# lgalke/aae-recommender

Hardware: AMD Instinct MI355X
Metric: train docs/sec at |items|=100k h=200 (higher is better)
Workload: dtype f32; 1 GPU; C3 PubMed-scale synthetic Bags: |items|=100000, hidden=200, code=50, fp32, batch=100 docs/GPU/step, full partial_fit (ae+disc+gen, 4 Adam) inside the AdversarialAutoEncoder.fit epoch loop (permutation batches of a corpus resident in HBM); n_items=100000, n_hidden=200, n_code=50, batch_per_gpu=100, global_batch=100, cond_inc=0, rng=device, parallelism=dp1

## Files before the change

### aae-recommender_amd/csrc/aae_abi.hip

```cpp
#include <hip/hip_runtime.h>
#include <hip/hip_ext.h>
#include <math.h>
#include <stdio.h>
#include <stdlib.h>
#include <string.h>

#include <algorithm>
#include <string>
#include <vector>

#include "../../include/aaerec_hip.h"
#include "gemm_f32.h"
#include "kernels.h"
#include "dec_fused.h"
#include "dec_fused_bf16.h"
#include "dec_crit_x3.h"
#include "rank_x3.h"
#include "chain.h"
#include "chain4.h"
#include "chain16x3.h"
#include "cond_embed.h"
#include "w1_update.h"

using namespace aae;
// ... 116 lines not shown
            m->bucket_wide_ok = hipFuncSetAttribute(reinterpret_cast<const void*>(tile_bucket_wide_kernel), hipFuncAttributeMaxDynamicSharedMemorySize, maxlds - 16384) == hipSuccess;
            {
                hipFuncAttributes fa;
                static bool told = false;
                if (m->bucket_wide_ok && !told && hipFuncGetAttributes(&fa, reinterpret_cast<const void*>(tile_bucket_wide_kernel)) == hipSuccess && fa.numRegs < 121) {
                    told = true;
                    fprintf(stderr, "aaerec: tile_bucket_wide_kernel allocates %d vector registers, not the 128 it claims to keep its CU to itself (buckets.h)\n", fa.numRegs);
                }
                (void)hipGetLastError();
            }
            if (e1 != hipSuccess || e2 != hipSuccess || e3 != hipSuccess || e4 != hipSuccess) m->fused_ok = false;
            if (m->bf16 &&
                (hipFuncSetAttribute(reinterpret_cast<const void*>(dec_fused_bf16_kernel<4>), hipFuncAttributeMaxDynamicSharedMemorySize, maxlds) != hipSuccess ||
                 hipFuncSetAttribute(reinterpret_cast<const void*>(dec_fused_bf16_kernel<7>), hipFuncAttributeMaxDynamicSharedMemorySize, maxlds) != hipSuccess ||
                 hipFuncSetAttribute(reinterpret_cast<const void*>(dec_fused_bf16_kernel<13>), hipFuncAttributeMaxDynamicSharedMemorySize, maxlds) != hipSuccess))
                m->fused_ok = false;
        }
    }
    m->late_enabled = !m->opt.no_late_join;
    m->early_enabled = true;
    m->early_any = m->opt.early_any;
    m->rank_ok = m->fused_ok && m->use_chain4 && !m->vae && !m->opt.no_rank_fused && rank_set_attributes();
    m->w1_big_lds = hipFuncSetAttribute(reinterpret_cast<const void*>(w1_item_update_kernel), hipFuncAttributeMaxDynamicSharedMemorySize,
                                        (int)(sizeof(int) * w1_items_lds_words(16384))) == hipSuccess;
    (void)hipGetLastError();
    m->grad_scale = 1.f;
    m->rng_row0 = 0; m->rng_global = 0;
    m->Gt = m->G.p;
    m->split_ok = false; m->opt_pending = false; m->side = nullptr; m->ev_crit = m->ev_opt = nullptr;
    m->split_wgs = std::max(1, (m->n_cu * 5) / 8);
    m->pf_armed = m->pf_built = m->pf_pending = false; m->pf_step = -1; m->hstep = 0; m->flushed_hstep = -1; m->ev_head = m->ev_pf = nullptr;
    bool side_ok = false;
    if (cfg->grad_mode == AAE_GRAD_FUSED) {
        int lo = 0, hi = 0;
        const unsigned evflags = hipEventDisableTiming | hipEventDisableSystemFence;
        side_ok = hipDeviceGetStreamPriorityRange(&lo, &hi) == hipSuccess &&
                  hipStreamCreateWithPriority(&m->side, hipStreamNonBlocking, lo) == hipSuccess &&
                  hipEventCreateWithFlags(&m->ev_crit, evflags) == hipSuccess &&
                  hipEventCreateWithFlags(&m->ev_opt, evflags) == hipSuccess &&
                  hipEventCreateWithFlags(&m->ev_head, evflags) == hipSuccess &&
                  hipEventCreateWithFlags(&m->ev_pf, evflags) == hipSuccess &&
                  hipEventCreateWithFlags(&m->ev_bk, evflags) == hipSuccess &&
                  hipEventCreateWithFlags(&m->ev_end, evflags) == hipSuccess;
        if (!side_ok) {
            if (m->side) (void)hipStreamDestroy(m->side);
            m->side = nullptr;
        }
        (void)hipGetLastError();
    }
    if (side_ok && m->fused_ok && m->bf16 && m->split_wgs > 0 &&
        (size_t)((m->N + kBU - 1) / kBU) * kBU * bf_stride(4) <= (size_t)m->R * m->ldn) {
        m->split_ok = hipFuncSetAttribute(reinterpret_cast<const void*>(dec_fused_bf16_kernel<4, kDecCrit>), hipFuncAttributeMaxDynamicSharedMemorySize, 160 * 1024) == hipSuccess
                && hipFuncSetAttribute(reinterpret_cast<const void*>(dec_fused_bf16_kernel<7, kDecCrit>), hipFuncAttributeMaxDynamicSharedMemorySize, 160 * 1024) == hipSuccess
                && hipFuncSetAttribute(reinterpret_cast<const void*>(dec_fused_bf16_kernel<13, kDecCrit>), hipFuncAttributeMaxDynamicSharedMemorySize, 160 * 1024) == hipSuccess
                && hipFuncSetAttribute(reinterpret_cast<const void*>(dec_fused_bf16_kernel<4, kDecOpt>), hipFuncAttributeMaxDynamicSharedMemorySize, 160 * 1024) == hipSuccess
                && hipFuncSetAttribute(reinterpret_cast<const void*>(dec_fused_bf16_kernel<7, kDecOpt>), hipFuncAttributeMaxDynamicSharedMemorySize, 160 * 1024) == hipSuccess
                && hipFuncSetAttribute(reinterpret_cast<const void*>(dec_fused_bf16_kernel<13, kDecOpt>), hipFuncAttributeMaxDynamicSharedMemorySize, 160 * 1024) == hipSuccess;
        (void)hipGetLastError();
    }
    if (side_ok && m->fused_ok && m->split_wgs > 0 && 
        (size_t)((m->N + kTI - 1) / kTI) * kTI * (size_t)std::min(m->R, 16 * kMB) * sizeof(float) < (size_t)0x7FFFFFF0u) {
        bool ok = true;
        ok = ok && aae_attr2(reinterpret_cast<const void*>(dec_fused_kernel<4, kDecCrit>), reinterpret_cast<const void*>(dec_fused_kernel<4, kDecCrit, true>), hipFuncAttributeMaxDynamicSharedMemorySize, 160 * 1024) == hipSuccess
                && aae_attr2(reinterpret_cast<const void*>(dec_fused_kernel<7, kDecCrit>), reinterpret_cast<const void*>(dec_fused_kernel<7, kDecCrit, true>), hipFuncAttributeMaxDynamicSharedMemorySize, 160 * 1024) == hipSuccess
                && aae_attr2(reinterpret_cast<const void*>(dec_fused_kernel<13, kDecCrit>), reinterpret_cast<const void*>(dec_fused_kernel<13, kDecCrit, true>), hipFuncAttributeMaxDynamicSharedMemorySize, 160 * 1024) == hipSuccess
                && aae_attr2(reinterpret_cast<const void*>(dec_fused_kernel<4, kDecOpt>), reinterpret_cast<const void*>(dec_fused_kernel<4, kDecOpt, true>), hipFuncAttributeMaxDynamicSharedMemorySize, 160 * 1024) == hipSuccess
                && aae_attr2(reinterpret_cast<const void*>(dec_fused_kernel<7, kDecOpt>), reinterpret_cast<const void*>(dec_fused_kernel<7, kDecOpt, true>), hipFuncAttributeMaxDynamicSharedMemorySize, 160 * 1024) == hipSuccess
                && aae_attr2(reinterpret_cast<const void*>(dec_fused_kernel<13, kDecOpt>), reinterpret_cast<const void*>(dec_fused_kernel<13, kDecOpt, true>), hipFuncAttributeMaxDynamicSharedMemorySize, 160 * 1024) == hipSuccess
                && aae_attr2(reinterpret_cast<const void*>(dec_fused_kernel<4, kDecOptAcc>), reinterpret_cast<const void*>(dec_fused_kernel<4, kDecOptAcc, true>), hipFuncAttributeMaxDynamicSharedMemorySize, 160 * 1024) == hipSuccess
                && aae_attr2(reinterpret_cast<const void*>(dec_fused_kernel<7, kDecOptAcc>), reinterpret_cast<const void*>(dec_fused_kernel<7, kDecOptAcc, true>), hipFuncAttributeMaxDynamicSharedMemorySize, 160 * 1024) == hipSuccess
                && aae_attr2(reinterpret_cast<const void*>(dec_fused_kernel<13, kDecOptAcc>), reinterpret_cast<const void*>(dec_fused_kernel<13, kDecOptAcc, true>), hipFuncAttributeMaxDynamicSharedMemorySize, 160 * 1024) == hipSuccess
                && hipFuncSetAttribute(reinterpret_cast<const void*>(dec_opt_blocks_kernel<4>), hipFuncAttributeMaxDynamicSharedMemorySize, 160 * 1024) == hipSuccess
                && hipFuncSetAttribute(reinterpret_cast<const void*>(dec_opt_blocks_kernel<7>), hipFuncAttributeMaxDynamicSharedMemorySize, 160 * 1024) == hipSuccess
                && hipFuncSetAttribute(reinterpret_cast<const void*>(dec_opt_blocks_kernel<13>), hipFuncAttributeMaxDynamicSharedMemorySize, 160 * 1024) == hipSuccess;
        if (!m->bf16) m->split_ok = ok;
        m->x3_ok = ok
                && aae_attr2(reinterpret_cast<const void*>(dec_crit_x3_kernel<4>), reinterpret_cast<const void*>(dec_crit_x3_kernel<4, false, false, true>), hipFuncAttributeMaxDynamicSharedMemorySize, 160 * 1024) == hipSuccess
                && aae_attr2(reinterpret_cast<const void*>(dec_crit_x3_kernel<7>), reinterpret_cast<const void*>(dec_crit_x3_kernel<7, false, false, true>), hipFuncAttributeMaxDynamicSharedMemorySize, 160 * 1024) == hipSuccess
                && aae_attr2(reinterpret_cast<const void*>(dec_crit_x3_kernel<13>), reinterpret_cast<const void*>(dec_crit_x3_kernel<13, false, false, true>), hipFuncAttributeMaxDynamicSharedMemorySize, 160 * 1024) == hipSuccess
                && hipFuncSetAttribute(reinterpret_cast<const void*>(dec_crit_x3_kernel<13, true>), hipFuncAttributeMaxDynamicSharedMemorySize, 160 * 1024) == hipSuccess
                && aae_attr2(reinterpret_cast<const void*>(dec_opt_blocks_x3_kernel<4>), reinterpret_cast<const void*>(dec_opt_blocks_x3_kernel<4, false, true>), hipFuncAttributeMaxDynamicSharedMemorySize, 160 * 1024) == hipSuccess
                && aae_attr2(reinterpret_cast<const void*>(dec_opt_blocks_x3_kernel<7>), reinterpret_cast<const void*>(dec_opt_blocks_x3_kernel<7, false, true>), hipFuncAttributeMaxDynamicSharedMemorySize, 160 * 1024) == hipSuccess
                && aae_attr2(reinterpret_cast<const void*>(dec_opt_blocks_x3_kernel<13>), reinterpret_cast<const void*>(dec_opt_blocks_x3_kernel<13, false, true>), hipFuncAttributeMaxDynamicSharedMemorySize, 160 * 1024) == hipSuccess
                && hipFuncSetAttribute(reinterpret_cast<const void*>(dec_opt_blocks_x3_kernel<13, true>), hipFuncAttributeMaxDynamicSharedMemorySize, 160 * 1024) == hipSuccess;
        (void)hipGetLastError();
        if (m->bf16) {
            m->bf16_x3 = m->x3_ok && ok;
            if (!m->bf16_x3) m->x3_ok = false;
            else m->split_ok = true;
            m->bf16_one = m->bf16_x3
                && aae_attr2(reinterpret_cast<const void*>(dec_crit_x3_kernel<4, false, true>), reinterpret_cast<const void*>(dec_crit_x3_kernel<4, false, true, true>), hipFuncAttributeMaxDynamicSharedMemorySize, 160 * 1024) == hipSuccess
                && aae_attr2(reinterpret_cast<const void*>(dec_crit_x3_kernel<7, false, true>), reinterpret_cast<const void*>(dec_crit_x3_kernel<7, false, true, true>), hipFuncAttributeMaxDynamicSharedMemorySize, 160 * 1024) == hipSuccess
                && aae_attr2(reinterpret_cast<const void*>(dec_crit_x3_kernel<13, false, true>), reinterpret_cast<const void*>(dec_crit_x3_kernel<13, false, true, true>), hipFuncAttributeMaxDynamicSharedMemorySize, 160 * 1024) == hipSuccess
                && aae_attr2(reinterpret_cast<const void*>(dec_opt_x3_kernel<4, true>), reinterpret_cast<const void*>(dec_opt_x3_kernel<4, true, true>), hipFuncAttributeMaxDynamicSharedMemorySize, 160 * 1024) == hipSuccess
                && aae_attr2(reinterpret_cast<const void*>(dec_opt_x3_kernel<7, true>), reinterpret_cast<const void*>(dec_opt_x3_kernel<7, true, true>), hipFuncAttributeMaxDynamicSharedMemorySize, 160 * 1024) == hipSuccess
                && aae_attr2(reinterpret_cast<const void*>(dec_opt_x3_kernel<13, true>), reinterpret_cast<const void*>(dec_opt_x3_kernel<13, true, true>), hipFuncAttributeMaxDynamicSharedMemorySize, 160 * 1024) == hipSuccess
                && aae_attr2(reinterpret_cast<const void*>(dec_opt_x3_kernel<4>), reinterpret_cast<const void*>(dec_opt_x3_kernel<4, false, true>), hipFuncAttributeMaxDynamicSharedMemorySize, 160 * 1024) == hipSuccess
                && aae_attr2(reinterpret_cast<const void*>(dec_opt_x3_kernel<7>), reinterpret_cast<const void*>(dec_opt_x3_kernel<7, false, true>), hipFuncAttributeMaxDynamicSharedMemorySize, 160 * 1024) == hipSuccess
                && aae_attr2(reinterpret_cast<const void*>(dec_opt_x3_kernel<13>), reinterpret_cast<const void*>(dec_opt_x3_kernel<13, false, true>), hipFuncAttributeMaxDynamicSharedMemorySize, 160 * 1024) == hipSuccess;
            (void)hipGetLastError();
        }
        if (m->x3_ok) {
            const int ntiles = (m->N + 31) / 32;
            const double t_tile = (3.3 + 0.0131 * m->h) * (m->bf16_one ? 0.87 : 1.0);
            int w = (int)(ntiles * t_tile / (m->bf16_one ? 165.0 : 82.0) / 8.0 + 0.5) * 8;
            w = std::max(w, std::min(ntiles, m->bf16_one ? 48 : 64));
            const int cap = m->late_enabled ? m->n_cu * 15 / 32 : m->n_cu * 9 / 16;
            m->split_wgs = std::max(1, std::min(w, cap));
        }
    }
    hipStream_t s = S(stream);
    hipError_t e = hipMemsetAsync(arena_dev, 0, need, s);
    if (e != hipSuccess) { delete m; return fail(AAE_EHIP, std::string("hipMemsetAsync: ") + hipGetErrorString(e)); }
    struct { Ten* t; int col; } ones[] = {{&m->eh1, m->h}, {&m->eh2, m->h}, {&m->zc, m->cp}, {&m->dh1, m->h},
                                           {&m->dh2, m->h}, {&m->zin, m->c}, {&m->xh1, m->h}, {&m->xh2, m->h}};
    for (auto& o : ones)
        hipLaunchKernelGGL(fill_col_kernel, dim3(((int)o.t->rows + 255) / 256), dim3(256), 0, s, o.t->p, (int)o.t->ld,
                           (int)o.t->rows, o.col, 1.0f);
    OptScalars hs[4]; memset(hs, 0, sizeof(hs));
    for (int i = 0; i < 4; ++i) {
        hs[i].t = 0; hs[i].is_sgd = cfg->optimizer == AAE_OPT_SGD;
        hs[i].lr = (i == O_ENC || i == O_DEC) ? (double)cfg->gen_lr : (double)cfg->reg_lr;
        hs[i].neg_step_size = 0.f; hs[i].bc2_sqrt = 1.f; hs[i].inv_bc2_sqrt = 1.f;
    }
    e = hipMemcpyAsync(m->sc, hs, sizeof(hs), hipMemcpyHostToDevice, s);
    if (e == hipSuccess) e = hipStreamSynchronize(s);
    if (e != hipSuccess) { delete m; return fail(AAE_EHIP, std::string("init: ") + hipGetErrorString(e)); }
    *out = m;
    return AAE_OK;
}

#ifdef W1_TS
int aae_debug_w1_ts(unsigned long long* out, int n) {
    return (int)hipMemcpyFromSymbol(out, HIP_SYMBOL(aae::w1_ts), sizeof(unsigned long long) * (size_t)n);
}
#endif
int aae_destroy(aae_handle h) {
    if (!h) return AAE_OK;
    if (h->side) {
        (void)hipStreamSynchronize(h->side);
        (void)hipStreamDestroy(h->side);
    }
    if (h->dp_scratch) (void)hipFree(h->dp_scratch);
    if (h->cnt_host) (void)hipHostFree(h->cnt_host);
    if (h->ev_crit) (void)hipEventDestroy(h->ev_crit);
    if (h->ev_opt) (void)hipEventDestroy(h->ev_opt);
    if (h->ev_head) (void)hipEventDestroy(h->ev_head);
    if (h->ev_pf) (void)hipEventDestroy(h->ev_pf);
    if (h->ev_bk) (void)hipEventDestroy(h->ev_bk);
    if (h->ev_end) (void)hipEventDestroy(h->ev_end);
    if (h->prof_ev) {
        for (int k = 0; k < AAE_K_N; ++k)
            for (auto& pr : h->prof_ev[k]) { (void)hipEventDestroy(pr.first); (void)hipEventDestroy(pr.second); }
        delete[] h->prof_ev;
    }
    delete h;
    return AAE_OK;
}


int aae_profile_enable(aae_handle h, int on) {
    if (!h) return fail(AAE_EINVAL, "handle is NULL");
    if (on && !h->prof_ev) h->prof_ev = new std::vector<std::pair<hipEvent_t, hipEvent_t>>[AAE_K_N];
    h->prof_on = on != 0;
    h->prof_mask = on == 1 ? ~0u : ((unsigned)on >> 1);
    return AAE_OK;
}
// ... 138 lines not shown
```

### aae-recommender_amd/csrc/abi_output_layer.h

```cpp
#pragma once

extern "C" {

int aae_ae_decode_backward(aae_handle m, const float* zc_dev, int64_t zc_ld, const aae_rng_inject* inj,
                           float* dzc_out, void* stream) {
    if (!m) return fail(AAE_EINVAL, "handle is NULL");
    if (m->phase != 1) return fail(AAE_ESTATE, "aae_ae_decode_backward without aae_ae_encode");
    remember_inject(m, inj, false);
    hipStream_t s = S(stream);
    const int B = m->rows, N = m->N, h = m->h, cp = m->cp;
    if (zc_dev) TRY(stage_zc(m, zc_dev, zc_ld, B, s));
    const uint8_t* mk2 = m->inj.masks_dev[2];
    const uint8_t* mk3 = m->inj.masks_dev[3];
    if (m->only_output_layer) {  }
    else if (m->use_chain) { if (!m->dec_hidden_done) TRY(chain_dec_hidden(m, true, B, s)); }
    else TRY(decoder_hidden_forward(m, true, mk2, mk3, B, s));
    TRY(join_output_layer(m, s));
    const float gscale = m->grad_scale / ((float)B * (float)N);
    DropSpec d1 = make_drop(m, 0, true, mk2, nullptr, B, h, 2);
    DropSpec d2 = make_drop(m, 1, true, mk3, nullptr, B, h, 3);
    const int nblk = m->have_batch ? row_blocks(m) : 1;
    const int Bb = (B + nblk - 1) / nblk;
    const bool win = x3_big_span(m->N, m->ldh);
    const size_t fused_lds = out_bf16(m) ? dec_fused_bf16_lds_bytes(m->fused_nb ? m->fused_nb : 13) : dec_fused_lds_bytes(Bb, h);
// ... 75 lines not shown
                        break;
                    }
                } else switch (m->fused_nb) {
                    case 4: { if (win) hipExtLaunchKernelGGL((dec_fused_kernel<4, kDecCrit, true>), dim3(grid), dim3(kNT), (uint32_t)fused_lds, s, start, stop, 0, b); else hipExtLaunchKernelGGL((dec_fused_kernel<4, kDecCrit>), dim3(grid), dim3(kNT), (uint32_t)fused_lds, s, start, stop, 0, b); } break;
                    case 7: { if (win) hipExtLaunchKernelGGL((dec_fused_kernel<7, kDecCrit, true>), dim3(grid), dim3(kNT), (uint32_t)fused_lds, s, start, stop, 0, b); else hipExtLaunchKernelGGL((dec_fused_kernel<7, kDecCrit>), dim3(grid), dim3(kNT), (uint32_t)fused_lds, s, start, stop, 0, b); } break;
                    default: { if (win) hipExtLaunchKernelGGL((dec_fused_kernel<13, kDecCrit, true>), dim3(grid), dim3(kNT), (uint32_t)fused_lds, s, start, stop, 0, b); else hipExtLaunchKernelGGL((dec_fused_kernel<13, kDecCrit>), dim3(grid), dim3(kNT), (uint32_t)fused_lds, s, start, stop, 0, b); } break;
                }
                LAUNCHCHK("dec_fused (critical launch)");
                if (r == nblk - 1) HIPCHK(hipStreamWaitEvent(m->side, stop, 0));
            }
            const int g2 = std::min(ntiles, std::min(m->split_wgs, m->n_cu));
            bool late_launched = false;
            constexpr bool no_obk = false, no_opt_x3 = false;
            const bool one_opt = nblk > 1 && !out_bf16(m) && !no_obk && ntiles <= kOBT * m->n_cu &&
                                 dec_opt_blocks_lds_bytes(Bb) <= 160 * 1024;
            constexpr bool no_obk_x3 = false;
            if (nblk > 1 && !out_bf16(m) && m->x3_ok && !no_opt_x3 && !no_obk_x3 && !no_obk && m->dh2f.p) {
                DecFusedArgs b = fa;
                b.nblk = nblk; b.Bb = Bb;
                hipLaunchKernelGGL(dh2_frag_kernel, dim3((B + kXCH - 1) / kXCH, m->fused_nb), dim3(128), 0, m->side, m->dh2.p, m->ldh, B,
                                   reinterpret_cast<u32x4_t*>(m->dh2f.p), b.one_term);
                b.acc = m->dh2f.p;
                const int wg_cap = ntiles >= 4096 ? m->n_cu * 7 / 8 : m->n_cu * 3 / 4;
                const int by_tiles = ntiles < 384 ? std::max(32, std::min(m->n_cu / 2, ntiles / 3))
                                                  : std::max(m->n_cu / 2, std::min(wg_cap, (int)(ntiles / 16.3 / 8.0 + 0.5) * 8));
                const int g3 = std::max(1, std::min(by_tiles, std::min(ntiles, m->n_cu)));
                const int rounds = (ntiles + g3 * kXBT - 1) / (g3 * kXBT);
                b.tpp = g3 * rounds;
                const uint32_t lds3 = (uint32_t)dec_opt_blocks_x3_lds_bytes();
                hipEvent_t start = nullptr, stop = nullptr;
                (void)prof_pair(m, AAE_K_DEC_OPT, &start, &stop);
                if (ts_obk && m->fused_nb == 13) {
                    hipExtLaunchKernelGGL((dec_opt_blocks_x3_kernel<13, true>), dim3(g3), dim3(kNT), lds3, m->side, start, stop, 0, b);
                    HIPCHK(hipStreamSynchronize(m->side));
                    unsigned long long t[128];
                    HIPCHK(hipMemcpy(t, ts_dev, sizeof(t), hipMemcpyDeviceToHost));
                    for (int w = 0; w < 2; ++w) {
                        fprintf(stderr, "[dec_opt_blocks_x3 wave %d, steps 8..15, us: products | split | to the next barrier;  spare wave: - | split | requests | wait for the slot | to the next barrier]", w ? 12 : 0);
                        for (int q = 0; q < 8; ++q) {
                            const unsigned long long* u = t + 64 * w + 4 * q;
                            if (w == 0) fprintf(stderr, "  %.2f %.2f %.2f", (u[1] - u[0]) * 0.01, (u[2] - u[1]) * 0.01, q < 7 ? ((double)u[4] - (double)u[2]) * 0.01 : 0.0);
                            else fprintf(stderr, "  %.2f %.2f %.2f %.2f", (u[1] - u[0]) * 0.01, (u[2] - u[1]) * 0.01, (u[3] - u[2]) * 0.01, q < 7 ? ((double)u[4] - (double)u[3]) * 0.01 : 0.0);
                        }
                        fprintf(stderr, "\n");
                    }
                    for (int k = 0; k < 2; ++k) {
                        const unsigned long long* u = t + (k ? 96 : 32);
                        fprintf(stderr, "[dec_opt_blocks_x3 step %d: every wave's arrival at the step's closing barrier, us after wave 0 finished its products]", k ? 12 : 9);
                        for (int w = 0; w < 16; ++w) fprintf(stderr, " %.2f", ((double)u[w] - (double)u[16]) * 0.01);
                        fprintf(stderr, "\n");
                    }
                } else
                switch (m->fused_nb) {
                    case 4: { if (win) hipExtLaunchKernelGGL((dec_opt_blocks_x3_kernel<4, false, true>), dim3(g3), dim3(kNT), lds3, m->side, start, stop, 0, b); else hipExtLaunchKernelGGL((dec_opt_blocks_x3_kernel<4>), dim3(g3), dim3(kNT), lds3, m->side, start, stop, 0, b); } break;
                    case 7: { if (win) hipExtLaunchKernelGGL((dec_opt_blocks_x3_kernel<7, false, true>), dim3(g3), dim3(kNT), lds3, m->side, start, stop, 0, b); else hipExtLaunchKernelGGL((dec_opt_blocks_x3_kernel<7>), dim3(g3), dim3(kNT), lds3, m->side, start, stop, 0, b); } break;
                    default: { if (win) hipExtLaunchKernelGGL((dec_opt_blocks_x3_kernel<13, false, true>), dim3(g3), dim3(kNT), lds3, m->side, start, stop, 0, b); else hipExtLaunchKernelGGL((dec_opt_blocks_x3_kernel<13>), dim3(g3), dim3(kNT), lds3, m->side, start, stop, 0, b); } break;
                }
                LAUNCHCHK("dec_opt_blocks_x3");
            } else if (one_opt) {
                DecFusedArgs b = fa;
                b.nblk = nblk; b.Bb = Bb;
                const int g3 = std::max(std::min(g2, ntiles), (ntiles + kOBT - 1) / kOBT);
                const uint32_t lds3 = (uint32_t)dec_opt_blocks_lds_bytes(Bb);
                hipEvent_t start = nullptr, stop = nullptr;
                (void)prof_pair(m, AAE_K_DEC_OPT, &start, &stop);
                switch (m->fused_nb) {
                    case 4: hipExtLaunchKernelGGL((dec_opt_blocks_kernel<4>), dim3(g3), dim3(kNT), lds3, m->side, start, stop, 0, b); break;
                    case 7: hipExtLaunchKernelGGL((dec_opt_blocks_kernel<7>), dim3(g3), dim3(kNT), lds3, m->side, start, stop, 0, b); break;
                    default: hipExtLaunchKernelGGL((dec_opt_blocks_kernel<13>), dim3(g3), dim3(kNT), lds3, m->side, start, stop, 0, b); break;
                }
                LAUNCHCHK("dec_opt_blocks");
            } else
            for (int r = 0; r < nblk; ++r) {
                DecFusedArgs b = block_args(r);
                if (nblk > 1) { b.acc = m->Gacc.p; b.gradV3 = r == nblk - 1 ? nullptr : m->Gacc.p; }
                hipEvent_t start = nullptr, stop = nullptr;
                (void)prof_pair(m, AAE_K_DEC_OPT, &start, &stop);
                if (out_bf16(m)) switch (m->fused_nb) {
                    case 4: hipExtLaunchKernelGGL((dec_fused_bf16_kernel<4, kDecOpt>), dim3(g2), dim3(kBT), (uint32_t)fused_lds, m->side, start, stop, 0, b); break;
                    case 7: hipExtLaunchKernelGGL((dec_fused_bf16_kernel<7, kDecOpt>), dim3(g2), dim3(kBT), (uint32_t)fused_lds, m->side, start, stop, 0, b); break;
                    default: hipExtLaunchKernelGGL((dec_fused_bf16_kernel<13, kDecOpt>), dim3(g2), dim3(kBT), (uint32_t)fused_lds, m->side, start, stop, 0, b); break;
                } else if (r == 0 && nblk == 1 && m->x3_ok && !no_opt_x3) {
                    const uint32_t lds_nat = (uint32_t)dec_opt_x3_lds_bytes();
                    const uint32_t lds3 = m->bf16_one ? std::max(lds_nat, 150u * 1024u) : lds_nat;
                    if (late) { b.dh2 = m->dh2s.p; b.sc = m->sc_snap; late_launched = true; }
                    if (m->bf16_one) switch (m->fused_nb) {
                    case 4: { if (win) hipExtLaunchKernelGGL((dec_opt_x3_kernel<4, true, true>), dim3(g2), dim3(kNT), lds3, m->side, start, stop, 0, b); else hipExtLaunchKernelGGL((dec_opt_x3_kernel<4, true>), dim3(g2), dim3(kNT), lds3, m->side, start, stop, 0, b); } break;
                    case 7: { if (win) hipExtLaunchKernelGGL((dec_opt_x3_kernel<7, true, true>), dim3(g2), dim3(kNT), lds3, m->side, start, stop, 0, b); else hipExtLaunchKernelGGL((dec_opt_x3_kernel<7, true>), dim3(g2), dim3(kNT), lds3, m->side, start, stop, 0, b); } break;
                    default: { if (win) hipExtLaunchKernelGGL((dec_opt_x3_kernel<13, true, true>), dim3(g2), dim3(kNT), lds3, m->side, start, stop, 0, b); else hipExtLaunchKernelGGL((dec_opt_x3_kernel<13, true>), dim3(g2), dim3(kNT), lds3, m->side, start, stop, 0, b); } break;
                    } else
                    switch (m->fused_nb) {
                    case 4: { if (win) hipExtLaunchKernelGGL((dec_opt_x3_kernel<4, false, true>), dim3(g2), dim3(kNT), lds3, m->side, start, stop, 0, b); else hipExtLaunchKernelGGL((dec_opt_x3_kernel<4>), dim3(g2), dim3(kNT), lds3, m->side, start, stop, 0, b); } break;
                    case 7: { if (win) hipExtLaunchKernelGGL((dec_opt_x3_kernel<7, false, true>), dim3(g2), dim3(kNT), lds3, m->side, start, stop, 0, b); else hipExtLaunchKernelGGL((dec_opt_x3_kernel<7>), dim3(g2), dim3(kNT), lds3, m->side, start, stop, 0, b); } break;
                    default: { if (win) hipExtLaunchKernelGGL((dec_opt_x3_kernel<13, false, true>), dim3(g2), dim3(kNT), lds3, m->side, start, stop, 0, b); else hipExtLaunchKernelGGL((dec_opt_x3_kernel<13>), dim3(g2), dim3(kNT), lds3, m->side, start, stop, 0, b); } break;
                    }
                } else if (r == 0) switch (m->fused_nb) {
                    case 4: { if (win) hipExtLaunchKernelGGL((dec_fused_kernel<4, kDecOpt, true>), dim3(g2), dim3(kNT), (uint32_t)fused_lds, m->side, start, stop, 0, b); else hipExtLaunchKernelGGL((dec_fused_kernel<4, kDecOpt>), dim3(g2), dim3(kNT), (uint32_t)fused_lds, m->side, start, stop, 0, b); } break;
                    case 7: { if (win) hipExtLaunchKernelGGL((dec_fused_kernel<7, kDecOpt, true>), dim3(g2), dim3(kNT), (uint32_t)fused_lds, m->side, start, stop, 0, b); else hipExtLaunchKernelGGL((dec_fused_kernel<7, kDecOpt>), dim3(g2), dim3(kNT), (uint32_t)fused_lds, m->side, start, stop, 0, b); } break;
                    default: { if (win) hipExtLaunchKernelGGL((dec_fused_kernel<13, kDecOpt, true>), dim3(g2), dim3(kNT), (uint32_t)fused_lds, m->side, start, stop, 0, b); else hipExtLaunchKernelGGL((dec_fused_kernel<13, kDecOpt>), dim3(g2), dim3(kNT), (uint32_t)fused_lds, m->side, start, stop, 0, b); } break;
                } else switch (m->fused_nb) {
                    case 4: { if (win) hipExtLaunchKernelGGL((dec_fused_kernel<4, kDecOptAcc, true>), dim3(g2), dim3(kNT), (uint32_t)fused_lds, m->side, start, stop, 0, b); else hipExtLaunchKernelGGL((dec_fused_kernel<4, kDecOptAcc>), dim3(g2), dim3(kNT), (uint32_t)fused_lds, m->side, start, stop, 0, b); } break;
                    case 7: { if (win) hipExtLaunchKernelGGL((dec_fused_kernel<7, kDecOptAcc, true>), dim3(g2), dim3(kNT), (uint32_t)fused_lds, m->side, start, stop, 0, b); else hipExtLaunchKernelGGL((dec_fused_kernel<7, kDecOptAcc>), dim3(g2), dim3(kNT), (uint32_t)fused_lds, m->side, start, stop, 0, b); } break;
                    default: { if (win) hipExtLaunchKernelGGL((dec_fused_kernel<13, kDecOptAcc, true>), dim3(g2), dim3(kNT), (uint32_t)fused_lds, m->side, start, stop, 0, b); else hipExtLaunchKernelGGL((dec_fused_kernel<13, kDecOptAcc>), dim3(g2), dim3(kNT), (uint32_t)fused_lds, m->side, start, stop, 0, b); } break;
                }
                LAUNCHCHK("dec_fused (optimiser launch)");
            }
            TRY(side_done(m, m->ev_opt));
            m->opt_pending = true;
            m->late_ok = late_launched;
            m->last_out_split = true; m->side_ordered = true;
            if (m->only_output_layer && m->pf_armed && m->mark2 && m->lazy) TRY(launch_prefetch(m, false));
        } else
        {
            m->last_out_split = false; m->side_ordered = false;
            ProfScope ps(m, AAE_K_DEC_FUSED, s);
            const size_t bf_lds = dec_fused_bf16_lds_bytes(m->fused_nb ? m->fused_nb : 13);
            if (m->bf16) switch (m->fused_nb) {
                case 4: hipLaunchKernelGGL(dec_fused_bf16_kernel<4>, dim3(grid), dim3(kBT), bf_lds, s, fa); break;
                case 7: hipLaunchKernelGGL(dec_fused_bf16_kernel<7>, dim3(grid), dim3(kBT), bf_lds, s, fa); break;
                default: hipLaunchKernelGGL(dec_fused_bf16_kernel<13>, dim3(grid), dim3(kBT), bf_lds, s, fa); break;
            } else switch (m->fused_nb) {
                case 4: { if (win) hipLaunchKernelGGL((dec_fused_kernel<4, kDecFused, true>), dim3(grid), dim3(kNT), fused_lds, s, fa); else hipLaunchKernelGGL((dec_fused_kernel<4>), dim3(grid), dim3(kNT), fused_lds, s, fa); } break;
                case 7: { if (win) hipLaunchKernelGGL((dec_fused_kernel<7, kDecFused, true>), dim3(grid), dim3(kNT), fused_lds, s, fa); else hipLaunchKernelGGL((dec_fused_kernel<7>), dim3(grid), dim3(kNT), fused_lds, s, fa); } break;
                default: { if (win) hipLaunchKernelGGL((dec_fused_kernel<13, kDecFused, true>), dim3(grid), dim3(kNT), fused_lds, s, fa); else hipLaunchKernelGGL((dec_fused_kernel<13>), dim3(grid), dim3(kNT), fused_lds, s, fa); } break;
            }
        }
        LAUNCHCHK("dec_fused");
        if (want_ts) {
            unsigned long long t[128];
            HIPCHK(hipStreamSynchronize(s));
            HIPCHK(hipMemcpy(t, ts_dev, sizeof(t), hipMemcpyDeviceToHost));
            if (m->last_out_split && ts_obk) {  }
            else if (m->last_out_split)
                fprintf(stderr, "[dec_crit_x3 tile 5] barrier=%.2f S0=%.2f GEMM1=%.2f BCE=%.2f GEMM3=%.2f | wg 0: prologue=%.2f loop=%.2f (%llu tiles, %.2f each) epilogue=%.2f us\n",
                        (t[14] - t[0]) * 0.01, (t[1] - t[14]) * 0.01, (t[2] - t[1]) * 0.01, (t[3] - t[2]) * 0.01, (t[4] - t[3]) * 0.01,
                        (t[11] - t[10]) * 0.01, (t[7] - t[11]) * 0.01, t[13], (t[7] - t[11]) * 0.01 / (double)(t[13] ? t[13] : 1),
                        (t[12] - t[7]) * 0.01);
            else {
            if (out_bf16(m))
                for (int k = 0; k < 5; ++k) {
                    fprintf(stderr, "[dec_fused_bf16 arrivals at barrier %d, us after the unit's start]", k);
                    for (int w = 0; w < 16; ++w) fprintf(stderr, " %.2f", ((double)t[16 + 16 * k + w] - (double)t[0]) * 0.01);
                    fprintf(stderr, "\n");
                }
            fprintf(stderr, "[dec_fused tile 5] S0=%.2f GEMM1+BCE0=%.2f entries=%.2f GEMM2+GEMM3=%.2f S5=%.2f | tile=%.2f us, %.0f shader clocks -> %.2f GHz\n",
                    (t[1] - t[0]) * 0.01, (t[2] - t[1]) * 0.01, (t[3] - t[2]) * 0.01, (t[4] - t[3]) * 0.01,
                    (t[6] - t[4]) * 0.01, (t[6] - t[0]) * 0.01, (double)(t[9] - t[8]),
                    (double)(t[9] - t[8]) / ((t[6] - t[0]) * 10.0));
            if (out_bf16(m)) fprintf(stderr, "[dec_fused_bf16 S0] barrier A=%.2f work=%.2f barrier B=%.2f us\n", (t[14] - t[0]) * 0.01, (t[15] - t[14]) * 0.01, (t[1] - t[15]) * 0.01);
            fprintf(stderr, "[dec_fused wg 0] prologue=%.2f loop=%.2f (%llu tiles, %.2f each) epilogue=%.2f us\n",
                    (t[11] - t[10]) * 0.01, (t[7] - t[11]) * 0.01, t[13], (t[7] - t[11]) * 0.01 / (double)(t[13] ? t[13] : 1),
                    (t[12] - t[7]) * 0.01);
            }
        }
        float* part = m->slabs.p + (size_t)304 * fa.slab_stride;
        const size_t n4 = (size_t)B * m->ldh / 4;
        if (m->only_output_layer && crit_slabs <= 64) {
            hipLaunchKernelGGL(slab_partial_kernel, dim3((unsigned)((n4 + 255) / 256), 1), dim3(256), 0, s, m->slabs.p, crit_slabs,
                               fa.slab_stride, n4, m->da2.p, (size_t)0, m->bce_partials, n_loss_partials,
                               1.0f / ((float)B * (float)N), m->losses, 0);
            LAUNCHCHK("slabs -> da2");
            m->phase = 2;
            return AAE_OK;
        }
        hipLaunchKernelGGL(slab_partial_kernel, dim3((unsigned)((n4 + 255) / 256), 16), dim3(256), 0, s, m->slabs.p, crit_slabs,
                           fa.slab_stride, n4, part, fa.slab_stride, m->bce_partials, n_loss_partials,
                           1.0f / ((float)B * (float)N), m->losses, 0);
        if (m->only_output_layer) {
            hipLaunchKernelGGL(slab_partial_kernel, dim3((unsigned)((n4 + 255) / 256), 1), dim3(256), 0, s, part, 16,
                               fa.slab_stride, n4, m->da2.p, (size_t)0, (const float*)nullptr, 0, 0.f, m->losses, 0);
            LAUNCHCHK("slab_partial -> da2");
            m->phase = 2;
            return AAE_OK;
        }
        if (m->use_chain) {
            chain_part = part; chain_stride = fa.slab_stride;
        } else {
// ... 112 lines not shown
```

### aae-recommender_amd/csrc/dec_crit_x3.h

```cpp
#pragma once
#include "dec_fused_bf16.h"

namespace aae {

typedef short s16x4_t __attribute__((ext_vector_type(4)));

__device__ __forceinline__ void split3_pair(float a, float b, unsigned& p1, unsigned& p2, unsigned& p3, bool one) {
    x3_split_pair(a, b, p1, p2, p3);
    if (one) { p2 = 0u; p3 = 0u; }
}
__device__ __forceinline__ f32x4 mfma_x3(const bf16x8 (&a)[3], const bf16x8 (&b)[3], f32x4 c) { return x3_mfma(a, b, c); }
template <bool ONE>
__device__ __forceinline__ f32x4 mfma_xt(const bf16x8 (&a)[3], const bf16x8 (&b)[3], f32x4 c) {
    if constexpr (ONE) return __builtin_amdgcn_mfma_f32_16x16x32_bf16(a[0], b[0], c, 0, 0, 0);
    else return x3_mfma(a, b, c);
}

__host__ __device__ constexpr int x3_stride(int kc) { return 16 * kc + 8; }
__device__ __forceinline__ bf16x8 x3_frag(const unsigned* img, int row, int S, int kc, int fk) {
    return __builtin_bit_cast(bf16x8, *reinterpret_cast<const u32x4_t*>(img + row * S + 16 * kc + 4 * fk));
}
constexpr int kXRS = 33;
constexpr int kXT = 32;

// ... 709 lines not shown
        for (int j = 0; j < kXBT; ++j) { acc[j][0] = (f32x4){0.f, 0.f, 0.f, 0.f}; acc[j][1] = (f32x4){0.f, 0.f, 0.f, 0.f}; }
        int q = 0;
        bf16x8 dB[KR][3];
        for (int ch = 0; ch < nch; ++ch) {
            if (mult && (ch == 0 || !(a.dbg_skip & 0x4000))) {
                const u32x4_t* F = reinterpret_cast<const u32x4_t*>(a.acc) + (((size_t)ch * NB + cb) * KR * 3) * 64 + lane;
#pragma unroll
                for (int kc = 0; kc < KR; ++kc)
#pragma unroll
                    for (int t = 0; t < 3; ++t) dB[kc][t] = __builtin_bit_cast(bf16x8, F[(kc * 3 + t) * 64]);
#pragma unroll
                for (int kc = 0; kc < KR; ++kc)
#pragma unroll
                    for (int t = 0; t < 3; ++t) {
                        u32x4_t v = __builtin_bit_cast(u32x4_t, dB[kc][t]);
                        asm volatile("" : "+v"(v));
                        dB[kc][t] = __builtin_bit_cast(bf16x8, v);
                    }
            }
#pragma unroll
            for (int j = 0; j < kXBT; ++j) {
                if (j >= nt) break;
                int oz;
                asm volatile("v_mov_b32 %0, 0" : "=v"(oz));
                const int lz = lane + oz;
                lds_barrier();
                const bool stamp = stamp_wg && (wave == 0 || wave == NM) && q >= 8 && q < 16;
                unsigned long long* tsq = a.ts + (wave ? 64 : 0) + (q - 8) * 4;
                if (stamp) tsq[0] = wall_clock64();
                if (mult && !(a.dbg_skip & 0x1000)) {
                    const int tq = (lz >> 2) & 3, tp = lz & 3, g = lz >> 4;
                    const unsigned* img = gB + (q & 1) * 3 * IMG;
#pragma unroll
                    for (int nb2 = 0; nb2 < 2; ++nb2) {
                        if (nb2 < nb_lo || nb2 >= nb_hi) continue;
                        f32x4 c = acc[j][nb2];
                        const unsigned* base = img + nb2 * (kXCH * 8) + (tq | ((g & 1) << 2) | ((g >> 1) << 4)) * 8 + 2 * tp;
#pragma unroll
                        for (int kc = 0; kc < KR; ++kc) {
                            bf16x8 ga[3];
#pragma unroll
                            for (int t = 0; t < 3; ++t) {
                                const unsigned* pb = base + t * IMG + 32 * kc * 8;
                                const s16x4_t lo = __builtin_amdgcn_ds_read_tr16_b64_v4i16((s16x4_t __attribute__((address_space(3)))*)(pb));
                                const s16x4_t hi = __builtin_amdgcn_ds_read_tr16_b64_v4i16((s16x4_t __attribute__((address_space(3)))*)(pb + 8 * 8));
                                typedef short s16x8_t __attribute__((ext_vector_type(8)));
                                const s16x8_t v = {lo[0], lo[1], lo[2], lo[3], hi[0], hi[1], hi[2], hi[3]};
                                ga[t] = __builtin_bit_cast(bf16x8, v);
                            }
                            c = mfma_x3(ga, dB[kc], c);
                        }
                        acc[j][nb2] = c;
                    }
                }
                if (stamp) tsq[1] = wall_clock64();
                if (splitter && q + 1 < Q) split_write(q + 1, j + 1 < nt ? ch : ch + 1, slot_read(q + 1));
                if (!mult) request(q + kXRing);
                if (stamp) tsq[2] = wall_clock64();
                if (!mult) {
                    asm volatile("s_waitcnt vmcnt(%0)" :: "n"(NS * (kXRing - 2)) : "memory");
                    if (stamp) tsq[3] = wall_clock64();
                }
                if (TS && stamp_wg && (q == 9 || q == 12)) { a.ts[(q == 9 ? 32 : 96) + wave] = wall_clock64(); if (wave == 0) a.ts[(q == 9 ? 48 : 112)] = tsq[1]; }
                ++q;
            }
        }
        asm volatile("s_waitcnt vmcnt(0)" ::: "memory");
        lds_barrier();
        if (mult) {
#pragma unroll
            for (int j = 0; j < kXBT; ++j)
#pragma unroll
                for (int nb2 = 0; nb2 < 2; ++nb2)
                    if (nb2 >= nb_lo && nb2 < nb_hi) {
#pragma unroll
                        for (int rr = 0; rr < 4; ++rr) os[j * (kTI * kSO) + (16 * nb2 + 4 * fk + rr) * kSO + 16 * cb + fr] = acc[j][nb2][rr];
                    }
        }
        lds_barrier();
        optimiser();
    }
}

}
```

Before: 434,100 docs/s.

## Add warp-specialized decoder optimiser kernel with dedicated loader waves prefetching tiles

```diff
diff --git a/aae-recommender_amd/csrc/aae_abi.hip b/aae-recommender_amd/csrc/aae_abi.hip
--- a/aae-recommender_amd/csrc/aae_abi.hip
+++ b/aae-recommender_amd/csrc/aae_abi.hip
@@ -222,7 +222,10 @@
                 && aae_attr2(reinterpret_cast<const void*>(dec_opt_blocks_x3_kernel<4>), reinterpret_cast<const void*>(dec_opt_blocks_x3_kernel<4, false, true>), hipFuncAttributeMaxDynamicSharedMemorySize, 160 * 1024) == hipSuccess
                 && aae_attr2(reinterpret_cast<const void*>(dec_opt_blocks_x3_kernel<7>), reinterpret_cast<const void*>(dec_opt_blocks_x3_kernel<7, false, true>), hipFuncAttributeMaxDynamicSharedMemorySize, 160 * 1024) == hipSuccess
                 && aae_attr2(reinterpret_cast<const void*>(dec_opt_blocks_x3_kernel<13>), reinterpret_cast<const void*>(dec_opt_blocks_x3_kernel<13, false, true>), hipFuncAttributeMaxDynamicSharedMemorySize, 160 * 1024) == hipSuccess
-                && hipFuncSetAttribute(reinterpret_cast<const void*>(dec_opt_blocks_x3_kernel<13, true>), hipFuncAttributeMaxDynamicSharedMemorySize, 160 * 1024) == hipSuccess;
+                && hipFuncSetAttribute(reinterpret_cast<const void*>(dec_opt_blocks_x3_kernel<13, true>), hipFuncAttributeMaxDynamicSharedMemorySize, 160 * 1024) == hipSuccess
+                && aae_attr2(reinterpret_cast<const void*>(dec_opt_ld_x3_kernel<4>), reinterpret_cast<const void*>(dec_opt_ld_x3_kernel<4, true>), hipFuncAttributeMaxDynamicSharedMemorySize, 160 * 1024) == hipSuccess
+                && aae_attr2(reinterpret_cast<const void*>(dec_opt_ld_x3_kernel<7>), reinterpret_cast<const void*>(dec_opt_ld_x3_kernel<7, true>), hipFuncAttributeMaxDynamicSharedMemorySize, 160 * 1024) == hipSuccess
+                && aae_attr2(reinterpret_cast<const void*>(dec_opt_ld_x3_kernel<13>), reinterpret_cast<const void*>(dec_opt_ld_x3_kernel<13, true>), hipFuncAttributeMaxDynamicSharedMemorySize, 160 * 1024) == hipSuccess;
         (void)hipGetLastError();
         if (m->bf16) {
             m->bf16_x3 = m->x3_ok && ok;
diff --git a/aae-recommender_amd/csrc/abi_output_layer.h b/aae-recommender_amd/csrc/abi_output_layer.h
--- a/aae-recommender_amd/csrc/abi_output_layer.h
+++ b/aae-recommender_amd/csrc/abi_output_layer.h
@@ -181,7 +181,7 @@
                     default: hipExtLaunchKernelGGL((dec_fused_bf16_kernel<13, kDecOpt>), dim3(g2), dim3(kBT), (uint32_t)fused_lds, m->side, start, stop, 0, b); break;
                 } else if (r == 0 && nblk == 1 && m->x3_ok && !no_opt_x3) {
                     const uint32_t lds_nat = (uint32_t)dec_opt_x3_lds_bytes();
-                    const uint32_t lds3 = m->bf16_one ? std::max(lds_nat, 150u * 1024u) : lds_nat;
+                    const uint32_t lds3 = m->bf16_one ? std::max(lds_nat, 150u * 1024u) : (uint32_t)dec_opt_ld_x3_lds_bytes();
                     if (late) { b.dh2 = m->dh2s.p; b.sc = m->sc_snap; late_launched = true; }
                     if (m->bf16_one) switch (m->fused_nb) {
                     case 4: { if (win) hipExtLaunchKernelGGL((dec_opt_x3_kernel<4, true, true>), dim3(g2), dim3(kNT), lds3, m->side, start, stop, 0, b); else hipExtLaunchKernelGGL((dec_opt_x3_kernel<4, true>), dim3(g2), dim3(kNT), lds3, m->side, start, stop, 0, b); } break;
@@ -189,9 +189,9 @@
                     default: { if (win) hipExtLaunchKernelGGL((dec_opt_x3_kernel<13, true, true>), dim3(g2), dim3(kNT), lds3, m->side, start, stop, 0, b); else hipExtLaunchKernelGGL((dec_opt_x3_kernel<13, true>), dim3(g2), dim3(kNT), lds3, m->side, start, stop, 0, b); } break;
                     } else
                     switch (m->fused_nb) {
-                    case 4: { if (win) hipExtLaunchKernelGGL((dec_opt_x3_kernel<4, false, true>), dim3(g2), dim3(kNT), lds3, m->side, start, stop, 0, b); else hipExtLaunchKernelGGL((dec_opt_x3_kernel<4>), dim3(g2), dim3(kNT), lds3, m->side, start, stop, 0, b); } break;
-                    case 7: { if (win) hipExtLaunchKernelGGL((dec_opt_x3_kernel<7, false, true>), dim3(g2), dim3(kNT), lds3, m->side, start, stop, 0, b); else hipExtLaunchKernelGGL((dec_opt_x3_kernel<7>), dim3(g2), dim3(kNT), lds3, m->side, start, stop, 0, b); } break;
-                    default: { if (win) hipExtLaunchKernelGGL((dec_opt_x3_kernel<13, false, true>), dim3(g2), dim3(kNT), lds3, m->side, start, stop, 0, b); else hipExtLaunchKernelGGL((dec_opt_x3_kernel<13>), dim3(g2), dim3(kNT), lds3, m->side, start, stop, 0, b); } break;
+                    case 4: { if (win) hipExtLaunchKernelGGL((dec_opt_ld_x3_kernel<4, true>), dim3(g2), dim3(kNT), lds3, m->side, start, stop, 0, b); else hipExtLaunchKernelGGL((dec_opt_ld_x3_kernel<4>), dim3(g2), dim3(kNT), lds3, m->side, start, stop, 0, b); } break;
+                    case 7: { if (win) hipExtLaunchKernelGGL((dec_opt_ld_x3_kernel<7, true>), dim3(g2), dim3(kNT), lds3, m->side, start, stop, 0, b); else hipExtLaunchKernelGGL((dec_opt_ld_x3_kernel<7>), dim3(g2), dim3(kNT), lds3, m->side, start, stop, 0, b); } break;
+                    default: { if (win) hipExtLaunchKernelGGL((dec_opt_ld_x3_kernel<13, true>), dim3(g2), dim3(kNT), lds3, m->side, start, stop, 0, b); else hipExtLaunchKernelGGL((dec_opt_ld_x3_kernel<13>), dim3(g2), dim3(kNT), lds3, m->side, start, stop, 0, b); } break;
                     }
                 } else if (r == 0) switch (m->fused_nb) {
                     case 4: { if (win) hipExtLaunchKernelGGL((dec_fused_kernel<4, kDecOpt, true>), dim3(g2), dim3(kNT), (uint32_t)fused_lds, m->side, start, stop, 0, b); else hipExtLaunchKernelGGL((dec_fused_kernel<4, kDecOpt>), dim3(g2), dim3(kNT), (uint32_t)fused_lds, m->side, start, stop, 0, b); } break;
diff --git a/aae-recommender_amd/csrc/dec_crit_x3.h b/aae-recommender_amd/csrc/dec_crit_x3.h
--- a/aae-recommender_amd/csrc/dec_crit_x3.h
+++ b/aae-recommender_amd/csrc/dec_crit_x3.h
@@ -815,4 +815,178 @@
     }
 }
 
-}
+constexpr int kXCW = 13;
+constexpr int kXSS = kTI * 16 * 13;
+constexpr int kXGF = 128 * kTI;
+
+inline size_t dec_opt_ld_x3_lds_bytes() {
+    return sizeof(float) * ((size_t)3 * 128 * kXGS + (size_t)kTI * kSO + (size_t)3 * kXSS + (size_t)kXGF + 64);
+}
+
+template <int NB, bool WIN = false>
+__global__ __launch_bounds__(kNT) void dec_opt_ld_x3_kernel(DecFusedArgs a) {
+    const bool one = a.one_term != 0;
+    constexpr int KR = 4;
+    constexpr int NCT = kXCW * 64;
+    constexpr int NV = 2;
+    static_assert(NB <= kXCW && kNT / 64 > kXCW, "one compute wave per column block, the rest load");
+    extern __shared__ __attribute__((aligned(16))) float lds[];
+    unsigned* gB = reinterpret_cast<unsigned*>(lds);
+    float* os = reinterpret_cast<float*>(gB + 3 * 128 * kXGS);
+    float* slot = os + kTI * kSO;
+    const int tid = threadIdx.x, lane = tid & 63;
+    const int wave = __builtin_amdgcn_readfirstlane(tid >> 6);
+    const bool loader = wave >= kXCW;
+    const int fr = lane & 15, fk = lane >> 4;
+    const int B = a.B, ldv = a.ldv, N = a.N;
+    const int ntiles = (N + kTI - 1) / kTI;
+    const int f4_per_row = ldv / 4, tile_f4 = kTI * f4_per_row;
+    const OptScalars sc = *a.sc;
+    const bool do_adam = a.gradV3 == nullptr;
+    typedef unsigned int fu32x4 __attribute__((ext_vector_type(4)));
+    if (a.dbg_skip & 0x10000) return;
+    if (a.dbg_skip & 0x20000) {
+        const unsigned long long t0 = wall_clock64();
+        while (wall_clock64() - t0 < 13500ull) __builtin_amdgcn_s_sleep(32);
+        return;
+    }
+
+    for (int i = tid; i < 3 * 128 * kXGS; i += kNT) gB[i] = 0u;
+
+    const int cb = min(wave, NB - 1);
+    const bool live = !loader && wave < NB;
+    bf16x8 dB[KR][3];
+    if (live) {
+        const int c = min(16 * cb + fr, a.ldh - 1);
+#pragma unroll
+        for (int kc = 0; kc < KR; ++kc) {
+            float x[8];
+#pragma unroll
+            for (int j = 0; j < 8; ++j) {
+                const int b = 32 * kc + 8 * fk + j;
+                x[j] = (b < B && 16 * cb + fr < a.ldh) ? a.dh2[(size_t)b * a.ldh + c] : 0.f;
+            }
+            unsigned p[3][4];
+#pragma unroll
+            for (int q = 0; q < 4; ++q) split3_pair(x[2 * q], x[2 * q + 1], p[0][q], p[1][q], p[2][q], one);
+#pragma unroll
+            for (int t = 0; t < 3; ++t) {
+                const u32x4_t v = {p[t][0], p[t][1], p[t][2], p[t][3]};
+                dB[kc][t] = __builtin_bit_cast(bf16x8, v);
+            }
+        }
+    }
+
+    const unsigned tile_bytes = (unsigned)(kTI * ldv) * 4u;
+    X3WindowT<WIN> win(N, ldv, tile_bytes);
+    const float* gbase = a.gradV3 ? a.gradV3 : a.V3a;
+    __amdgpu_buffer_rsrc_t rP = win.desc(a.V3a), rM = win.desc(a.M), rV = win.desc(a.V), rG = win.desc(gbase);
+    const int g_f4 = B * (kTI / 4);
+
+    const int lw = wave - kXCW;
+    const unsigned slot_lds = (unsigned)reinterpret_cast<size_t>(slot);
+    auto request = [&](int t) {
+        const int nv = min(kTI, N - t * kTI) * f4_per_row;
+        const size_t e0 = (size_t)t * kTI * ldv;
+        const float* src[3] = {a.V3a + e0, a.M + e0, a.V + e0};
+#pragma unroll
+        for (int s = 0; s < 3; ++s)
+            for (int q = lw; 64 * q < nv; q += kNT / 64 - kXCW)
+                if (64 * q + lane < nv) glds16(src[s] + 4 * (64 * q + lane), __builtin_amdgcn_readfirstlane(slot_lds + 4u * (unsigned)(s * kXSS) + 1024u * q));
+        const float* g = a.Gt + (size_t)t * g_f4 * 4;
+        for (int q = lw; 64 * q < g_f4; q += kNT / 64 - kXCW)
+            if (64 * q + lane < g_f4) glds16(g + 4 * (64 * q + lane), __builtin_amdgcn_readfirstlane(slot_lds + 4u * (unsigned)(3 * kXSS) + 1024u * q));
+    };
+
+    int s_rc[NV];
+#pragma unroll
+    for (int j = 0; j < NV; ++j) {
+        const int fc = min(tid + NCT * j, tile_f4 - 1), row = fc / f4_per_row;
+        s_rc[j] = row * 64 + (fc - row * f4_per_row);
+    }
+    const unsigned lane_off = (unsigned)tid * 16u;
+    int tile = blockIdx.x;
+    const int stride = gridDim.x;
+    if (loader && tile < ntiles) {
+        request(tile);
+        asm volatile("s_waitcnt vmcnt(0)" ::: "memory");
+    }
+    lds_barrier();
+
+    for (; tile < ntiles; tile += stride) {
+        const int i0 = tile * kTI;
+        if (win.moves(tile)) { rP = win.desc(a.V3a); rM = win.desc(a.M); rV = win.desc(a.V); rG = win.desc(gbase); }
+        int oz;
+        asm volatile("v_mov_b32 %0, 0" : "=v"(oz));
+        const int lz = lane + oz;
+        float4 p_cur[NV], mreg[NV], sreg[NV];
+        if (!loader) {
+#pragma unroll
+            for (int j = 0; j < NV; ++j) {
+                const float4* s4 = reinterpret_cast<const float4*>(slot) + tid + NCT * j;
+                p_cur[j] = s4[0]; mreg[j] = s4[kXSS / 4]; sreg[j] = s4[2 * (kXSS / 4)];
+            }
+            for (int f = tid; f < g_f4; f += NCT) {
+                const float4 x = reinterpret_cast<const float4*>(slot + 3 * kXSS)[f];
+                unsigned q0[3], q1[3];
+                split3_pair(x.x, x.y, q0[0], q0[1], q0[2], one);
+                split3_pair(x.z, x.w, q1[0], q1[1], q1[2], one);
+                unsigned* d = gB + (f >> 3) * kXGS + (f & 7) * 2;
+#pragma unroll
+                for (int t = 0; t < 3; ++t) *reinterpret_cast<uint2*>(d + t * (128 * kXGS)) = make_uint2(q0[t], q1[t]);
+            }
+        }
+        lds_barrier();
+
+        if (loader) {
+            if (tile + stride < ntiles) request(tile + stride);
+        } else if (live) {
+            const int tq = (lz >> 2) & 3, tp = lz & 3, g = lz >> 4;
+            for (int nb2 = 0; nb2 < 2; ++nb2) {
+                f32x4 c = (f32x4){0.f, 0.f, 0.f, 0.f};
+                const unsigned* base = gB + (8 * g + tq) * kXGS + 8 * nb2 + 2 * tp;
+#pragma unroll
+                for (int kc = 0; kc < KR; ++kc) {
+                    bf16x8 ga[3];
+#pragma unroll
+                    for (int t = 0; t < 3; ++t) {
+                        const unsigned* pb = base + t * (128 * kXGS) + 32 * kc * kXGS;
+                        const s16x4_t lo = __builtin_amdgcn_ds_read_tr16_b64_v4i16((s16x4_t __attribute__((address_space(3)))*)(pb));
+                        const s16x4_t hi = __builtin_amdgcn_ds_read_tr16_b64_v4i16((s16x4_t __attribute__((address_space(3)))*)(pb + 4 * kXGS));
+                        typedef short s16x8_t __attribute__((ext_vector_type(8)));
+                        const s16x8_t v = {lo[0], lo[1], lo[2], lo[3], hi[0], hi[1], hi[2], hi[3]};
+                        ga[t] = __builtin_bit_cast(bf16x8, v);
+                    }
+                    c = mfma_xt<false>(ga, dB[kc], c);
+                }
+#pragma unroll
+                for (int r = 0; r < 4; ++r) os[(16 * nb2 + 4 * fk + r) * kSO + 16 * cb + fr] = c[r];
+            }
+        }
+        lds_barrier();
+
+        if (loader) {
+            asm volatile("s_waitcnt vmcnt(0)" ::: "memory");
+        } else {
+            const int nv = min(kTI, N - i0) * f4_per_row;
+#pragma unroll
+            for (int j = 0; j < NV; ++j) {
+                const bool valid = tid + NCT * j < nv;
+                const float4 g = *reinterpret_cast<const float4*>(os + (s_rc[j] >> 6) * kSO + (s_rc[j] & 63) * 4);
+                const unsigned so = win.so(tile);
+                const unsigned vo = valid ? lane_off + (unsigned)(NCT * 16 * j) : 0x80000000u;
+                float4 p = p_cur[j], mm = mreg[j], vv = sreg[j];
+                adam_update(p.x, mm.x, vv.x, g.x, sc); adam_update(p.y, mm.y, vv.y, g.y, sc);
+                adam_update(p.z, mm.z, vv.z, g.z, sc); adam_update(p.w, mm.w, vv.w, g.w, sc);
+                const float4 out = do_adam ? p : g;
+                const unsigned vo2 = (do_adam && !sc.is_sgd) ? vo : 0x80000000u;
+                __builtin_amdgcn_raw_buffer_store_b128(__builtin_bit_cast(fu32x4, out), do_adam ? rP : rG, vo, so, 2);
+                __builtin_amdgcn_raw_buffer_store_b128(__builtin_bit_cast(fu32x4, mm), rM, vo2, so, 2);
+                __builtin_amdgcn_raw_buffer_store_b128(__builtin_bit_cast(fu32x4, vv), rV, vo2, so, 2);
+            }
+        }
+        lds_barrier();
+    }
+}
+
+}
```

Measured after the change: 437,300 docs/s, median of 6. Within noise of the previous version (+0.7%).
